# nighting0le01/On_Device_Image_Captioning

Measured on AMD Instinct MI355X. Metric: captions/sec end-to-end (Swin-L 384, beam=3) at 1/2/4/8 MI355X, higher is better.
Workload: dtype bf16; 1 GPU; End_ExpansionNet_v2 end-to-end, Swin-L/384 backbone, batch 16 per GPU, beam 3, beam_max_seq_len 20 (BASELINE.json configs[2]); workload_key=e2e16, batch_per_gpu=16, beam=3, beam_max_seq_len=20, decoder_steps=19, weights=synthetic xavier (Philox, seed 0), backbone_precision=bf16, encoder_precision=bf16, decoder_precision=fp32, hip_graphs=True, parallelism=image-shard x1, caption_len_check=20, encode_lanes=1, decode_lanes=2, decode_cus=0, decode_group_batches=1

## Files before the change

include/odic_hip.h:

```cpp
#ifndef ODIC_HIP_H
#define ODIC_HIP_H

#include <stddef.h>
#include <stdint.h>

#ifdef __cplusplus
extern "C" {
#endif

#define ODIC_F32 0
#define ODIC_BF16 1
#define ODIC_FP8 2
#define ODIC_F16 3
#define ODIC_H2 4

#define ODIC_ACT_NONE 0
#define ODIC_ACT_GELU 1
#define ODIC_ACT_RELU 2
#define ODIC_ACT_SIGMOID 3

#define ODIC_EINVAL (-1)
#define ODIC_ENULL (-2)
#define ODIC_EUNSUPPORTED (-3)

#define ODIC_ABI_VERSION 22
int odic_abi_version(void);

const char* odic_build_info(void);

typedef struct odic_gemm_args {
  const void* A; const void* W; const float* bias; const float* residual; void* out;
  int32_t M, N, K;
  int64_t lda, ldw, ldr, ldc;
  int32_t batch;
  int64_t strideA, strideW, strideBias, strideR, strideC;
  float alpha;
  int32_t act;
  int32_t bias_axis;
  int32_t in_dtype;
  int32_t out_dtype;
  int32_t tile_cfg;
  const float* ln_colsum; float ln_eps;
  int32_t* workspace;
  const float* col_scale; float out_scale;
  void* out16; int64_t ld16; float* stats_out;
  const float* ln_stats;
  const float* a_ln; int64_t ld_aln;
} odic_gemm_args;
int odic_gemm(const odic_gemm_args* args, void* stream);

int odic_layernorm(const float* x, int64_t ldx, const float* gamma, const float* beta, void* out,
                   int32_t M, int32_t C, float eps, int32_t out_dtype, void* stream);

int odic_copy(const void* src, void* dst, int64_t nbytes, void* stream);

int odic_cast_f32_to_bf16(const float* x, int64_t ldx, void* out, int64_t ldo, int32_t M, int32_t C,
                          void* stream);
int odic_cast_f32_to_h2(const float* x, int64_t ldx, void* out, int64_t ldo, int32_t M, int32_t C, void* stream);

int odic_patch_merge_layernorm(const float* x, const float* gamma, const float* beta, void* out,
                               int32_t B, int32_t res, int32_t C, float eps, int32_t out_dtype,
                               void* stream);

int odic_patch_embed(const float* img, const float* w, const float* b, const float* gamma,
                     const float* beta, float* out, int32_t B, int32_t in_chans, int32_t H,
                     int32_t W, int32_t patch, int32_t C, float eps, void* stream);

int odic_resize_bilinear_normalize(const uint8_t* src_rgb, int32_t H, int32_t W, int64_t src_stride_bytes,
                                   const int32_t* bounds_x, const int32_t* coef_x, int32_t ksize_x,
                                   const int32_t* bounds_y, const int32_t* coef_y, int32_t ksize_y,
                                   uint8_t* tmp, float* dst, int32_t out_size, const float* mean3,
                                   const float* std3, void* stream);

typedef struct odic_resize_job {
  int64_t src_off, src_pitch, tmp_off;
  int32_t H, W, row_first, n_rows;
  int32_t bounds_x, coef_x, bounds_y, coef_y;
  int32_t ksize_x, ksize_y;
// ... 36 lines not shown
#define ODIC_JPEG_MAX_SCANS 64

typedef struct odic_jpeg_table {
  uint16_t lut[512];
  int32_t maxcode[18];
  int32_t valoff[18];
  uint8_t huffval[256];
} odic_jpeg_table;

typedef struct odic_jpeg_prog_header {
  int64_t out_off, coef_off, plane_off;
  int32_t width, height, sampling, mcus_x, mcus_y, n_intervals;
  uint16_t qt[3][64];
} odic_jpeg_prog_header;

typedef struct odic_jpeg_scan {
  int64_t data_off, data_end, scan_off;
  int32_t image, int_off, n_intervals, restart, n_units, blocks_w, comp_mask, ss, se, ah, al, level;
  int32_t table[3];
  int32_t pad;
} odic_jpeg_scan;

typedef struct odic_jpeg_prog_batch {
  const void* headers;
  const void* scans;
  const void* tables;
  const uint8_t* data;
  uint8_t* out;
  int32_t* status;
  int32_t n_images, n_scans, n_tables, n_levels, max_width, max_height, pad0, pad1;
  int64_t max_blocks, total_scan_bytes, total_intervals, total_blocks, total_plane_bytes;
  int32_t level_first[ODIC_JPEG_MAX_SCANS + 1];
  int32_t level_intervals[ODIC_JPEG_MAX_SCANS];
  int32_t pad2;
} odic_jpeg_prog_batch;

size_t odic_jpeg_progressive_workspace_bytes(const odic_jpeg_prog_batch* batch);

size_t odic_jpeg_progressive_coef_offset(const odic_jpeg_prog_batch* batch);

int odic_jpeg_decode_progressive(const odic_jpeg_prog_batch* batch, void* workspace, size_t ws_bytes, void* stream);

int odic_jpeg_decode_progressive_scaled(const odic_jpeg_prog_batch* batch, const int32_t* scale_log2, void* workspace,
                                        size_t ws_bytes, void* stream);

int odic_window_attention(const void* qkv, const float* bias_table, const float* bias_shifted_prescaled,
                          void* out, int32_t B, int32_t res, int32_t C, int32_t heads, int32_t ws,
                          int32_t shift, float scale, int32_t dtype, void* stream);

int odic_swin_qkv_attention(const float* x, int64_t ldx, const void* w_qkv_folded, const float* b_qkv_folded,
                            const float* bias_shifted_prescaled, void* out, int32_t B, int32_t res, int32_t C,
                            int32_t heads, int32_t ws, int32_t shift, float scale, float ln_eps, void* stream);

int odic_stcexp_normalize(const float* z, const int32_t* enc_len, const int32_t* group_meta,
                          int32_t ngroups, void* pos_fw, void* neg_fw, int64_t ld_fw, void* pos_bw,
                          void* neg_bw, int64_t ld_bw, float* colsum_ws, int32_t B, int32_t nq,
                          int32_t S, float eps, float scale_fw, float scale_bw, int32_t out_dtype, void* stream);

int odic_selector_mix(const float* x, int64_t ldx, const float* sel_pre, int64_t lds,
                      const float* a, int64_t lda, const float* b, int64_t ldb, float* out,
                      int64_t ldo, int32_t M, int32_t d, void* stream);


int odic_dec_embed(const int64_t* tokens, const float* embed, const float* pos_table,
                   const int32_t* pos, float* y, int64_t ldy, int32_t N, int32_t d, int32_t pos_rows,
                   float scale, void* stream);

int odic_dynexp_step(const float* lin, int64_t ldlin, const float* qexp, const float* bexp,
                     float* cond_c, float* key_c, float* va_c, float* vb_c, float* wfa_c,
                     float* wfb_c, float* qk_c, const int32_t* anc, const int32_t* row_valid,
                     const int32_t* pos, const float* y_in, int64_t ldy_in, float* y, int64_t ldy,
                     int32_t N, int32_t T, int32_t d, int32_t E, float eps, void* stream);


int odic_dec_embed_seq(const int64_t* tokens, const float* embed, const float* pos_table, const int32_t* dec_len,
                       int32_t* row_valid, float* y, int64_t ldy, int32_t N, int32_t T, int32_t d, int32_t vocab,
                       int32_t pos_rows, float scale, void* stream);

int odic_dynexp_seq(const float* lin, int64_t ldlin, const float* qexp, const float* bexp, const int32_t* dec_len,
                    const float* y_in, int64_t ldy_in, float* y, int64_t ldy, int32_t N, int32_t T, int32_t d,
                    int32_t E, float eps, void* stream);

int odic_token_stats(const float* logits, int64_t ldl, const int64_t* target, float* logp_target, float* sum_logp,
                     int32_t* argmax, float* max_logp, int32_t* status, int32_t R, int32_t V, void* stream);

int odic_cross_attn_step(const float* q, int64_t ldq, const float* kv, int64_t ldkv, int32_t koff,
                         int32_t voff, const int32_t* enc_len, const int32_t* row_valid, float* out,
                         int64_t ldo, int32_t N, int32_t n_img, int32_t S, int32_t d, int32_t heads,
                         void* stream);

int odic_cross_attn_probs(const float* q, int64_t ldq, const float* kv, int64_t ldkv, int32_t koff,
                          const int32_t* enc_len, const int32_t* row_valid, float* out, int64_t ldo,
                          int32_t N, int32_t n_img, int32_t S, int32_t d, int32_t heads,
                          int32_t per_head, int32_t accumulate, float scale, void* stream);

int odic_logsoftmax_topk(const float* logits, int64_t ldl, float* logp_out, int64_t ldp,
                         float* top_val, int32_t* top_idx, int32_t N, int32_t V, int32_t k,
                         void* stream);

int odic_logsoftmax_sample(const float* logits, int64_t ldl, float* logp_out, int64_t ldp, float* top_val,
                           int32_t* top_idx, int32_t N, int32_t V, int32_t k, uint64_t seed,
                           const int32_t* pos, void* stream);

int odic_ensemble_logprobs(const float* const* logits, int32_t M, int64_t ldl, float* out, int64_t ldo,
                           int32_t N, int32_t V, void* stream);
int odic_topk_rows(const float* logp, int64_t ldl, float* top_val, int32_t* top_idx, int32_t N, int32_t V,
// ... 30 lines not shown
```

on_device_image_captioning_amd/_hip.py:

```python
from __future__ import annotations

import ctypes as C
import os

_HERE = os.path.dirname(os.path.abspath(__file__))
LIB_PATH = os.path.join(_HERE, "libodic_hip.so")

F32, BF16, FP8, F16, H2 = 0, 1, 2, 3, 4
ACT_NONE, ACT_GELU, ACT_RELU, ACT_SIGMOID = 0, 1, 2, 3
ABI_VERSION = 22

_ERR = {-1: "ODIC_EINVAL (bad shape / alignment / enum)", -2: "ODIC_ENULL (required pointer is NULL)",
        -3: "ODIC_EUNSUPPORTED"}


class GemmArgs(C.Structure):
    _fields_ = [("A", C.c_void_p), ("W", C.c_void_p), ("bias", C.c_void_p), ("residual", C.c_void_p),
                ("out", C.c_void_p),
                ("M", C.c_int32), ("N", C.c_int32), ("K", C.c_int32),
                ("lda", C.c_int64), ("ldw", C.c_int64), ("ldr", C.c_int64), ("ldc", C.c_int64),
                ("batch", C.c_int32),
                ("strideA", C.c_int64), ("strideW", C.c_int64), ("strideBias", C.c_int64),
                ("strideR", C.c_int64), ("strideC", C.c_int64),
                ("alpha", C.c_float), ("act", C.c_int32), ("bias_axis", C.c_int32),
                ("in_dtype", C.c_int32), ("out_dtype", C.c_int32), ("tile_cfg", C.c_int32),
                ("ln_colsum", C.c_void_p), ("ln_eps", C.c_float), ("workspace", C.c_void_p),
                ("col_scale", C.c_void_p), ("out_scale", C.c_float),
                ("out16", C.c_void_p), ("ld16", C.c_int64), ("stats_out", C.c_void_p), ("ln_stats", C.c_void_p),
                ("a_ln", C.c_void_p), ("ld_aln", C.c_int64)]


class BeamState(C.Structure):
    _fields_ = [(n, C.c_void_p) for n in
                ("tokens", "logprobs", "anc", "cumul", "n_elem", "has_eos", "row_valid", "next_tok",
                 "pos", "done", "ctr")]


class EmbedArgs(C.Structure):
    _fields_ = [("embed", C.c_void_p), ("pos_table", C.c_void_p), ("y", C.c_void_p), ("ldy", C.c_int64),
                ("d", C.c_int32), ("scale", C.c_float), ("pos_rows", C.c_int32)]


class JpegBatch(C.Structure):
    _fields_ = [("headers", C.c_void_p), ("data", C.c_void_p), ("out", C.c_void_p), ("status", C.c_void_p),
                ("n_images", C.c_int32), ("subseq_bits", C.c_int32), ("max_sync_passes", C.c_int32),
                ("max_units", C.c_int32), ("max_intervals", C.c_int32), ("max_width", C.c_int32),
                ("max_height", C.c_int32), ("pad", C.c_int32),
                ("max_blocks", C.c_int64), ("max_scan_bytes", C.c_int64), ("total_scan_bytes", C.c_int64),
                ("total_intervals", C.c_int64), ("total_units", C.c_int64), ("total_blocks", C.c_int64),
                ("total_plane_bytes", C.c_int64)]


JPEG_MAX_SCANS = 64


class JpegProgBatch(C.Structure):
    _fields_ = [("headers", C.c_void_p), ("scans", C.c_void_p), ("tables", C.c_void_p), ("data", C.c_void_p),
                ("out", C.c_void_p), ("status", C.c_void_p),
                ("n_images", C.c_int32), ("n_scans", C.c_int32), ("n_tables", C.c_int32), ("n_levels", C.c_int32),
                ("max_width", C.c_int32), ("max_height", C.c_int32), ("pad0", C.c_int32), ("pad1", C.c_int32),
                ("max_blocks", C.c_int64), ("total_scan_bytes", C.c_int64), ("total_intervals", C.c_int64),
                ("total_blocks", C.c_int64), ("total_plane_bytes", C.c_int64),
                ("level_first", C.c_int32 * (JPEG_MAX_SCANS + 1)), ("level_intervals", C.c_int32 * JPEG_MAX_SCANS),
                ("pad2", C.c_int32)]


_P, _I32, _I64, _F = C.c_void_p, C.c_int32, C.c_int64, C.c_float

_SIGNATURES = {
    "odic_abi_version": (C.c_int, []),
    "odic_build_info": (C.c_char_p, []),
    "odic_gemm": (C.c_int, [C.POINTER(GemmArgs), _P]),
    "odic_layernorm": (C.c_int, [_P, _I64, _P, _P, _P, _I32, _I32, _F, _I32, _P]),
    "odic_cast_f32_to_bf16": (C.c_int, [_P, _I64, _P, _I64, _I32, _I32, _P]),
    "odic_cast_f32_to_h2": (C.c_int, [_P, _I64, _P, _I64, _I32, _I32, _P]),
    "odic_patch_merge_layernorm": (C.c_int, [_P, _P, _P, _P, _I32, _I32, _I32, _F, _I32, _P]),
    "odic_patch_embed": (C.c_int, [_P] * 6 + [_I32] * 6 + [_F, _P]),
    "odic_resize_bilinear_normalize": (C.c_int, [_P, _I32, _I32, _I64, _P, _P, _I32, _P, _P, _I32, _P, _P, _I32,
                                                 C.POINTER(C.c_float), C.POINTER(C.c_float), _P]),
    "odic_resize_boxes_normalize": (C.c_int, [_P, _I32, _P, _P, _P, _P, C.c_size_t, _P, _I32, _I32,
                                              C.POINTER(C.c_float), C.POINTER(C.c_float), _P]),
    "odic_window_attention": (C.c_int, [_P, _P, _P, _P] + [_I32] * 6 + [_F, _I32, _P]),
    "odic_swin_qkv_attention": (C.c_int, [_P, _I64, _P, _P, _P, _P] + [_I32] * 6 + [_F, _F, _P]),
    "odic_stcexp_normalize": (C.c_int, [_P, _P, _P, _I32, _P, _P, _I64, _P, _P, _I64, _P, _I32, _I32, _I32, _F, _F, _F, _I32,
                                        _P]),
    "odic_selector_mix": (C.c_int, [_P, _I64, _P, _I64, _P, _I64, _P, _I64, _P, _I64, _I32, _I32, _P]),
    "odic_copy": (C.c_int, [_P, _P, _I64, _P]),
    "odic_dec_embed": (C.c_int, [_P, _P, _P, _P, _P, _I64, _I32, _I32, _I32, _F, _P]),
    "odic_dec_embed_seq": (C.c_int, [_P, _P, _P, _P, _P, _P, _I64] + [_I32] * 5 + [_F, _P]),
    "odic_dynexp_seq": (C.c_int, [_P, _I64, _P, _P, _P, _P, _I64, _P, _I64] + [_I32] * 4 + [_F, _P]),
    "odic_token_stats": (C.c_int, [_P, _I64, _P, _P, _P, _P, _P, _P, _I32, _I32, _P]),
    "odic_dynexp_step": (C.c_int, [_P, _I64, _P, _P] + [_P] * 7 + [_P, _P, _P, _P, _I64, _P, _I64] + [_I32] * 4 + [_F, _P]),
    "odic_cross_attn_step": (C.c_int, [_P, _I64, _P, _I64, _I32, _I32, _P, _P, _P, _I64] + [_I32] * 5 + [_P]),
    "odic_cross_attn_probs": (C.c_int, [_P, _I64, _P, _I64, _I32, _P, _P, _P, _I64] + [_I32] * 7 + [_F, _P]),
    "odic_logsoftmax_topk": (C.c_int, [_P, _I64, _P, _I64, _P, _P, _I32, _I32, _I32, _P]),
    "odic_logsoftmax_sample": (C.c_int, [_P, _I64, _P, _I64, _P, _P, _I32, _I32, _I32, C.c_uint64, _P, _P]),
    "odic_ensemble_logprobs": (C.c_int, [C.POINTER(C.c_void_p), _I32, _I64, _P, _I64, _I32, _I32, _P]),
    "odic_topk_rows": (C.c_int, [_P, _I64, _P, _P, _I32, _I32, _I32, _P]),
    "odic_beam_step": (C.c_int, [_P, _P, C.POINTER(BeamState), C.POINTER(EmbedArgs), _I32, _I32, _I32, _I64, _P]),
    "odic_beam_finalize": (C.c_int, [C.POINTER(BeamState), _P, _P, _I32, _I32, _P]),
    "odic_beam_finalize_best": (C.c_int, [C.POINTER(BeamState), _P, _P, _P, _P, _I32, _I32, _I32, _I32, _P]),
    "odic_beam_reset": (C.c_int, [C.POINTER(BeamState), C.POINTER(EmbedArgs), _I32, _I32, _I32, _I64, _P]),
    "odic_jpeg_workspace_bytes": (C.c_size_t, [C.POINTER(JpegBatch)]),
    "odic_jpeg_decode": (C.c_int, [C.POINTER(JpegBatch), _P, C.c_size_t, _P]),
    "odic_jpeg_progressive_workspace_bytes": (C.c_size_t, [C.POINTER(JpegProgBatch)]),
    "odic_jpeg_progressive_coef_offset": (C.c_size_t, [C.POINTER(JpegProgBatch)]),
    "odic_jpeg_decode_progressive": (C.c_int, [C.POINTER(JpegProgBatch), _P, C.c_size_t, _P]),
    "odic_jpeg_decode_scaled": (C.c_int, [C.POINTER(JpegBatch), _P, _P, C.c_size_t, _P]),
    "odic_jpeg_decode_progressive_scaled": (C.c_int, [C.POINTER(JpegProgBatch), _P, _P, C.c_size_t, _P]),
}

EXPORTED_SYMBOLS = tuple(_SIGNATURES)

_lib = None


def load() -> C.CDLL:
    global _lib
    if _lib is not None:
        return _lib
    if not os.path.exists(LIB_PATH):
        raise RuntimeError(
            f"{LIB_PATH} is missing: the HIP extension is not built and there is no CPU fallback. "
            "Run `python -c 'import __graft_entry__ as g; g.build()'` from the repository root.")
    lib = C.CDLL(LIB_PATH)
    for name, (res, args) in _SIGNATURES.items():
        fn = getattr(lib, name)
        fn.restype = res
        fn.argtypes = args
    got = lib.odic_abi_version()
    if got != ABI_VERSION:
        raise RuntimeError(f"libodic_hip.so ABI {got} != binding ABI {ABI_VERSION}; rebuild")
    _lib = lib
    return lib


# ... 7 lines not shown
```

on_device_image_captioning_amd/csrc/gemm_bf16.hip:

```cpp
#include "gemm_tile.h"
#include <stdio.h>
#include <stdlib.h>
#include <type_traits>

namespace {

struct Params {
  const bf16_raw* A; const bf16_raw* W; const float* bias; const float* residual; void* out;
  int M, N, K;
  long lda, ldw, ldr, ldc;
  long strideA, strideW, strideBias, strideR, strideC;
  float alpha; int act; int bias_axis;
  TileGrid grid;
  const float* a_ln; long ld_aln; float ln_eps;
};

template <int NWM, int NWN, int MI, int NI, int NSTAGE, int BK, typename OutT, int KS = 1>
__global__ __launch_bounds__(64 * NWM * NWN * KS, (NWM * NWN * KS == 4 && MI * NI == 32) ? 2 : 1) void gemm_bf16_nt_kernel(Params p) {
  static_assert(KS == 1 || (KS == 2 && BK == 64), "the K-split form is two groups on 64-deep K-tiles");
  constexpr int NW = NWM * NWN;
  constexpr int ROWB = BK * 2;
  constexpr int RPI = 1024 / ROWB;
  constexpr int CPR = ROWB / 16;
  constexpr int BM = NWM * MI * 16, BN = NWN * NI * 16;
// ... 514 lines not shown
    } else {
#pragma unroll
      for (int nq = 0; nq < NI / 2; ++nq) {
#pragma unroll
        for (int mi = 0; mi < MI; ++mi) {
          f32x4_t v[2];
          finish(mi, nq, v);
          OutT* dst = out + (long)(m0 + (wave * MI + mi) * 16 + frow) * p.ldc + c * BNC + nq * 32 + fq * 8;
          if constexpr (sizeof(OutT) == 4) {
            ((f32x4_t*)dst)[0] = v[0]; ((f32x4_t*)dst)[1] = v[1];
          } else {
            bf16x8_t pk;
#pragma unroll
            for (int e = 0; e < 4; ++e) { pk[e] = (short)f32_to_bf16(v[0][e]); pk[4 + e] = (short)f32_to_bf16(v[1][e]); }
            *(bf16x8_t*)dst = pk;
          }
        }
      }
    }
  }
}

template <int MI, int NI, int KT, int KH = 1>
int launch_apanel(Params& p, int out_dtype, int batch, hipStream_t stream) {
  constexpr int BM = 4 * MI * 16, BNC = NI * 16;
  if (batch != 1 || p.K != KT * 64 || p.M % BM != 0 || p.N % BNC != 0 || p.bias_axis != 0)
    return ODIC_EUNSUPPORTED;
  if ((long)BNC * p.ldw >= (1L << 30) || (p.residual && MI > 2))
    return ODIC_EUNSUPPORTED;
  if ((p.ldc & 7) || ((uintptr_t)p.out & 15) || (p.residual && ((p.ldr & 3) || ((uintptr_t)p.residual & 15))))
    return ODIC_EUNSUPPORTED;
  const int panels = p.M / BM, nchunks = p.N / BNC;
  static const int want = getenv("ODIC_APANEL_BLOCKS") ? atoi(getenv("ODIC_APANEL_BLOCKS")) : 1536;
  const int nsplit = panel_split(panels, nchunks, want);
  dim3 grid(8 * ((panels + 7) / 8) * nsplit), block(256);
  const int SHMEM = 2 * (KT / KH) * BNC * 128 + (nchunks + nsplit - 1) / nsplit * BNC * 4;
  if (SHMEM > 64 * 1024) return ODIC_EUNSUPPORTED;
  if (p.a_ln) {
    if (p.residual || (p.ld_aln & 3) || ((uintptr_t)p.a_ln & 15)) return ODIC_EUNSUPPORTED;
    if (out_dtype == ODIC_BF16) hipLaunchKernelGGL((gemm_bf16_apanel_kernel<MI, NI, KT, KH, bf16_raw, false, true>), grid, block, SHMEM, stream, p, nsplit);
    else hipLaunchKernelGGL((gemm_bf16_apanel_kernel<MI, NI, KT, KH, float, false, true>), grid, block, SHMEM, stream, p, nsplit);
    return odic_launch_status();
  }
  if constexpr (MI <= 2) {
    if (p.residual) {
      if (out_dtype == ODIC_BF16) hipLaunchKernelGGL((gemm_bf16_apanel_kernel<MI, NI, KT, KH, bf16_raw, true>), grid, block, SHMEM, stream, p, nsplit);
      else hipLaunchKernelGGL((gemm_bf16_apanel_kernel<MI, NI, KT, KH, float, true>), grid, block, SHMEM, stream, p, nsplit);
      return odic_launch_status();
    }
  }
  if (out_dtype == ODIC_BF16) hipLaunchKernelGGL((gemm_bf16_apanel_kernel<MI, NI, KT, KH, bf16_raw, false>), grid, block, SHMEM, stream, p, nsplit);
  else hipLaunchKernelGGL((gemm_bf16_apanel_kernel<MI, NI, KT, KH, float, false>), grid, block, SHMEM, stream, p, nsplit);
  return odic_launch_status();
}

template <int NWM, int NWN, int MI, int NI, int NSTAGE, int BK = 64, int KS = 1>
int launch_cfg(Params& p, int out_dtype, int batch, hipStream_t stream) {
  constexpr int BM = NWM * MI * 16, BN = NWN * NI * 16;
  constexpr int SH_STAGES = NSTAGE * (BM + BN) * BK * 2 + BM * 8;
  constexpr int SH_RED = KS == 2 ? NWM * NWN * MI * NI * 1024 : 0;
  constexpr int SHMEM = SH_STAGES > SH_RED ? SH_STAGES : SH_RED;
  if (p.K % BK != 0) return ODIC_EINVAL;
  const int max_rect = tile_grid(p.grid, p.M, p.N, BM, BN, (double)p.M * p.K * 2.0, (double)p.N * p.K * 2.0,
                                 32 * (NWM * NWN * KS <= 4 ? 2 : 1));
  dim3 grid(8 * max_rect, 1, batch), block(64 * NWM * NWN * KS);
  constexpr auto kb = gemm_bf16_nt_kernel<NWM, NWN, MI, NI, NSTAGE, BK, bf16_raw, KS>;
  constexpr auto kf = gemm_bf16_nt_kernel<NWM, NWN, MI, NI, NSTAGE, BK, float, KS>;
  tile_allow_lds<SHMEM, kb, kf>();
  if (out_dtype == ODIC_BF16) hipLaunchKernelGGL(kb, grid, block, SHMEM, stream, p);
  else hipLaunchKernelGGL(kf, grid, block, SHMEM, stream, p);
  return odic_launch_status();
}


}

int odic_gemm_bf16_launch(const odic_gemm_args* a, hipStream_t stream) {
  if (a->ln_colsum) return ODIC_EUNSUPPORTED;
  if (a->K % 64 != 0 || (a->A && a->lda % 8 != 0) || a->ldw % 8 != 0) return ODIC_EINVAL;
  if (((uintptr_t)a->A & 15) || ((uintptr_t)a->W & 15)) return ODIC_EINVAL;
  if (a->a_ln && (a->tile_cfg < 50 || a->tile_cfg > 53)) return ODIC_EUNSUPPORTED;
  if (!a->a_ln && !a->A) return ODIC_EINVAL;
  if ((a->strideA % 8) || (a->strideW % 8)) return ODIC_EINVAL;
  Params p;
  p.A = (const bf16_raw*)a->A; p.W = (const bf16_raw*)a->W; p.bias = a->bias; p.residual = a->residual;
  p.out = a->out; p.M = a->M; p.N = a->N; p.K = a->K;
  p.lda = a->lda; p.ldw = a->ldw; p.ldr = a->ldr; p.ldc = a->ldc;
  p.strideA = a->strideA; p.strideW = a->strideW; p.strideBias = a->strideBias;
  p.strideR = a->strideR; p.strideC = a->strideC;
  p.alpha = a->alpha; p.act = a->act; p.bias_axis = a->bias_axis;
  p.a_ln = a->a_ln; p.ld_aln = a->ld_aln; p.ln_eps = a->ln_eps;
  int cfg = a->tile_cfg;
  if (cfg < 0) {
    const double c0 = tile_rounds(a->M, a->N, a->batch, 128, 64, 768) * 1.0;
    const double c1 = tile_rounds(a->M, a->N, a->batch, 128, 128, 512) * 1.38;
    const double c2 = a->N % 256 == 0 ? tile_rounds(a->M, a->N, a->batch, 256, 256, 256) * 2.6 : 1e30;
    cfg = (c0 <= c1 && c0 <= c2) ? 0 : (c1 <= c2 ? 1 : 2);
  }
  switch (cfg) {
    case 0: return launch_cfg<2, 2, 4, 2, 2>(p, a->out_dtype, a->batch, stream);
    case 1: return launch_cfg<2, 2, 4, 4, 2>(p, a->out_dtype, a->batch, stream);
    case 2: return launch_cfg<2, 4, 8, 4, 2>(p, a->out_dtype, a->batch, stream);
    case 7: return launch_cfg<4, 2, 4, 4, 2, 32>(p, a->out_dtype, a->batch, stream);
    case 10: return launch_cfg<4, 2, 4, 4, 3, 32>(p, a->out_dtype, a->batch, stream);
    case 40: return launch_cfg<6, 2, 3, 6, 2, 64>(p, a->out_dtype, a->batch, stream);
    case 41: return launch_cfg<3, 3, 3, 6, 2, 64>(p, a->out_dtype, a->batch, stream);
    case 42: return launch_cfg<3, 2, 3, 6, 2, 64>(p, a->out_dtype, a->batch, stream);
    case 43: return launch_cfg<3, 2, 3, 6, 3, 64>(p, a->out_dtype, a->batch, stream);
    case 44: return launch_cfg<3, 1, 3, 6, 2, 64>(p, a->out_dtype, a->batch, stream);
    case 45: return launch_cfg<3, 3, 3, 6, 3, 32>(p, a->out_dtype, a->batch, stream);
    case 46: return launch_cfg<3, 1, 3, 6, 3, 64>(p, a->out_dtype, a->batch, stream);
    case 47: return launch_cfg<3, 2, 3, 6, 2, 64, 2>(p, a->out_dtype, a->batch, stream);
    case 48: return launch_cfg<2, 2, 2, 2, 3, 64>(p, a->out_dtype, a->batch, stream);
    case 49: return launch_cfg<2, 2, 2, 2, 2, 64>(p, a->out_dtype, a->batch, stream);
    case 50: return launch_apanel<4, 4, 3>(p, a->out_dtype, a->batch, stream);
    case 51: return launch_apanel<2, 2, 6>(p, a->out_dtype, a->batch, stream);
    case 52: return launch_apanel<2, 4, 3>(p, a->out_dtype, a->batch, stream);
    case 53: return launch_apanel<2, 4, 6, 2>(p, a->out_dtype, a->batch, stream);
    default: return ODIC_EINVAL;
  }
}
```

on_device_image_captioning_amd/engine.py:

```python
from __future__ import annotations

import ctypes as C
import math
import os
from typing import Dict, List, Optional, Sequence, Tuple

import torch

from . import _hip, ops
from .weights import Geometry

SD = Dict[str, torch.Tensor]
_CDT = {"fp32": torch.float32, "bf16": torch.bfloat16, "fp8": torch.bfloat16, "x3": ops.H2_DTYPE}


def pack_operand(t: torch.Tensor, cdt) -> Tuple[torch.Tensor, float]:
    if cdt == ops.H2_DTYPE:
        sc = ops.pow2_scale_for_h2(t)
        return ops.h2_from_f32(t * sc), 1.0 / sc
    return t.to(cdt).contiguous(), 1.0


def _dev(t: torch.Tensor, device, dtype=None) -> torch.Tensor:
    t = t.detach()
    if dtype is not None and t.dtype != dtype:
        t = t.to(dtype)
    return t.to(device).contiguous()


class SwinEngine:
    def __init__(self, sd: SD, g: Geometry, device, precision: str = "fp32", calibration_images=None):
        if precision not in _CDT:
            raise ValueError(f"precision must be one of {list(_CDT)}")
        self.g, self.device, self.precision = g, device, precision
        self.cdt = _CDT[precision]
        fp8 = precision == "fp8"
        fast_attn = precision in ("bf16", "fp8", "x3")
        P = "swin_transf"
        f32 = lambda k: _dev(sd[k], device, torch.float32)
        cw = lambda k: pack_operand(_dev(sd[k], device, torch.float32), self.cdt)
        self.pe_w = _dev(sd[f"{P}.patch_embed.proj.weight"].reshape(g.swin_embed_dim, -1), device, torch.float32)
        self.pe_b = f32(f"{P}.patch_embed.proj.bias")
        self.pe_g, self.pe_beta = f32(f"{P}.patch_embed.norm.weight"), f32(f"{P}.patch_embed.norm.bias")
        self.stages = []
        for s, depth in enumerate(g.swin_depths):
            blocks = []
            for b in range(depth):
                p = f"{P}.layers.{s}.blocks.{b}"
                (qkv_w, qkv_a), (proj_w, proj_a) = cw(p + ".attn.qkv.weight"), cw(p + ".attn.proj.weight")
                (fc1_w, fc1_a), (fc2_w, fc2_a) = cw(p + ".mlp.fc1.weight"), cw(p + ".mlp.fc2.weight")
                blocks.append(dict(
                    n1w=f32(p + ".norm1.weight"), n1b=f32(p + ".norm1.bias"),
                    qkv_w=qkv_w, qkv_a=qkv_a, qkv_b=f32(p + ".attn.qkv.bias"),
                    table=f32(p + ".attn.relative_position_bias_table"),
                    dense=(ops.shifted_bias_prescaled(f32(p + ".attn.relative_position_bias_table"), g.stage_window(s),
                                                      (g.stage_dim(s) // g.swin_num_heads[s]) ** -0.5)
                           if fast_attn and g.stage_window(s) == 12 else None),
                    proj_w=proj_w, proj_a=proj_a, proj_b=f32(p + ".attn.proj.bias"),
                    n2w=f32(p + ".norm2.weight"), n2b=f32(p + ".norm2.bias"),
                    fc1_w=fc1_w, fc1_a=fc1_a, fc1_b=f32(p + ".mlp.fc1.bias"),
                    fc2_w=fc2_w, fc2_a=fc2_a, fc2_b=f32(p + ".mlp.fc2.bias"),
                    shift=g.stage_shift(s, b)))
            down = None
            if s < len(g.swin_depths) - 1:
                p = f"{P}.layers.{s}.downsample"
                red_w, red_a = cw(p + ".reduction.weight")
                down = dict(nw=f32(p + ".norm.weight"), nb=f32(p + ".norm.bias"), red_w=red_w, red_a=red_a)
            self.stages.append((blocks, down))
        self.fn_w, self.fn_b = f32(f"{P}.norm.weight"), f32(f"{P}.norm.bias")
        self.stage_chunks = [int(v) for v in os.environ.get("ODIC_SWIN_CHUNKS", "1").split(",")]
        lr = os.environ.get("ODIC_FUSE_BACKBONE_LN_READ", "1")
        self.ln_read = (precision == "bf16" and lr != "0") or (precision == "x3" and lr == "x3")
        self.fuse_qkv_attn = precision == "bf16" and os.environ.get("ODIC_FUSE_QKV_ATTENTION", "1") == "1"
        if self.ln_read:
            for s, (blocks, _) in enumerate(self.stages):
                if g.stage_dim(s) != 192:
                    continue
                for b, w in enumerate(blocks):
                    p = f"{P}.layers.{s}.blocks.{b}"
                    if precision == "bf16":
                        w["qkv_lnr"] = ops.fold_layernorm_bf16(f32(p + ".attn.qkv.weight"), w["qkv_b"], w["n1w"], w["n1b"])[:2] + (1.0,)
                        w["fc1_lnr"] = ops.fold_layernorm_bf16(f32(p + ".mlp.fc1.weight"), w["fc1_b"], w["n2w"], w["n2b"])[:2] + (1.0,)
                    else:
                        for name, wk, bk, nw, nb in (("qkv_lnr", ".attn.qkv.weight", "qkv_b", "n1w", "n1b"),
                                                     ("fc1_lnr", ".mlp.fc1.weight", "fc1_b", "n2w", "n2b")):
                            Wg, b2, _ = ops.fold_layernorm(f32(p + wk), w[bk], w[nw], w[nb])
                            op, alpha = pack_operand(Wg, self.cdt)
                            w[name] = (op, b2, alpha)
        self.fp8_ready = False
        if fp8:
            self._pack_fp8(sd, calibration_images)

    def _pack_fp8(self, sd: SD, calibration_images) -> None:
        from .weights import synth_images
        g, dv = self.g, self.device
        if any(g.stage_window(s) != 12 or g.stage_dim(s) % 64 for s in range(len(g.swin_depths))):
            raise RuntimeError("fp8 mode needs 12x12 windows and stage widths that are multiples of 64 (Swin-L: 192·2^s)")
        img = calibration_images if calibration_images is not None else synth_images(2, g, seed=7)
        amax = {}
        self.forward(img.to(dv, torch.float32), _amax=amax)
        P = "swin_transf"
        margin = 1.25
        self.fp8_range = {k: margin * v for k, v in amax.items()}
        for s, (blocks, _) in enumerate(self.stages):
            for b, w in enumerate(blocks):
                p = f"{P}.layers.{s}.blocks.{b}"
                s1 = margin * amax[(s, b, "ln1")] / ops.FP8_MAX
                s2 = margin * amax[(s, b, "ln2")] / ops.FP8_MAX
                sh = margin * amax[(s, b, "hid")] / ops.FP8_MAX
                f32 = lambda k: _dev(sd[k], dv, torch.float32)
                q_qkv, sw_qkv = ops.quantize_fp8_per_channel(f32(p + ".attn.qkv.weight"))
                q_fc1, sw_fc1 = ops.quantize_fp8_per_channel(f32(p + ".mlp.fc1.weight"))
                q_fc2, sw_fc2 = ops.quantize_fp8_per_channel(f32(p + ".mlp.fc2.weight"))
                w.update(dict(
                    n1w8=(w["n1w"] / s1).contiguous(), n1b8=(w["n1b"] / s1).contiguous(),
                    n2w8=(w["n2w"] / s2).contiguous(), n2b8=(w["n2b"] / s2).contiguous(),
                    qkv_w8=q_qkv, qkv_cs=(sw_qkv * s1).contiguous(),
                    fc1_w8=q_fc1, fc1_cs=(sw_fc1 * s2).contiguous(), hid_inv=1.0 / sh,
                    fc2_w8=q_fc2, fc2_cs=(sw_fc2 * sh).contiguous(),
                    proj_w16=f32(p + ".attn.proj.weight").to(torch.float16).contiguous()))
        self.fp8_ready = True

    def fp8_saturation(self, img: torch.Tensor) -> dict:
        if not self.fp8_ready:
            raise RuntimeError("not an fp8 engine")
        seen = {}
        self.forward(img, _amax=seen)
        ratios = {k: seen[k] / self.fp8_range[k] for k in seen}
        over = {f"s{k[0]}b{k[1]}.{k[2]}": round(v, 3) for k, v in ratios.items() if v > 1.0}
        return {"tensors": len(ratios), "clipping_tensors": len(over), "worst_ratio": round(max(ratios.values()), 3),
                "median_ratio": round(sorted(ratios.values())[len(ratios) // 2], 3), "clipping": over}

    def forward(self, img: torch.Tensor, taps: Optional[dict] = None, out_dtype=torch.float32,
                _amax: Optional[dict] = None) -> torch.Tensor:
        g, cdt = self.g, self.cdt
        if img.dtype != torch.float32 or not img.is_cuda:
            raise RuntimeError("SwinEngine.forward wants an fp32 CUDA image batch")
        img = img.contiguous()
        B = img.shape[0]
        fp8 = self.fp8_ready and _amax is None
        x = ops.patch_embed(img, self.pe_w, self.pe_b, self.pe_g, self.pe_beta, g.swin_patch_size)
        if taps is not None:
            taps["patch_embed"] = x.clone()
        for s, (blocks, down) in enumerate(self.stages):
            res, C_, heads, ws = g.stage_res(s), g.stage_dim(s), g.swin_num_heads[s], g.stage_window(s)
            x = x.view(B * res * res, C_)
            n_ch = self.stage_chunks[s] if s < len(self.stage_chunks) else 1
            if taps is not None or _amax is not None or n_ch < 1 or B % n_ch:
                n_ch = 1
            x_all, B_all = x, B
            B = B_all // n_ch
            for ci, bi, w in ((ci, bi, w) for ci in range(n_ch) for bi, w in enumerate(blocks)):
                x = x_all[ci * B * res * res:(ci + 1) * B * res * res]
                if fp8:
                    xn = ops.layernorm(x, w["n1w8"], w["n1b8"], out_dtype=ops.FP8_DTYPE)
                    qkv = ops.gemm(xn, w["qkv_w8"], w["qkv_b"], col_scale=w["qkv_cs"], out_dtype=torch.float16)
                    att = ops.window_attention(qkv, w["table"], B, res, C_, heads, ws, w["shift"],
                                               bias_shifted_prescaled=w["dense"])
                    ops.gemm(att, w["proj_w16"], w["proj_b"], residual=x, out=x)
                    xn = ops.layernorm(x, w["n2w8"], w["n2b8"], out_dtype=ops.FP8_DTYPE)
                    h = ops.gemm(xn, w["fc1_w8"], w["fc1_b"], act=ops.ACT_GELU, col_scale=w["fc1_cs"],
                                 out_scale=w["hid_inv"], out_dtype=ops.FP8_DTYPE)
                    ops.gemm(h, w["fc2_w8"], w["fc2_b"], residual=x, out=x, col_scale=w["fc2_cs"])
                elif "qkv_lnr" in w and _amax is None and ops.a_ln_supported(x.shape[0], 3 * C_, C_, cdt):
                    if self.fuse_qkv_attn and ws == 12 and w["dense"] is not None:
                        att = ops.swin_qkv_attention(x, w["qkv_lnr"][0], w["qkv_lnr"][1], w["dense"], B, res, C_, heads,
                                                     ws, w["shift"])
                    else:
                        qkv = ops.gemm(None, w["qkv_lnr"][0], w["qkv_lnr"][1], a_ln=x, out_dtype=cdt, alpha=w["qkv_lnr"][2])
                        att = ops.window_attention(qkv, w["table"], B, res, C_, heads, ws, w["shift"],
                                                   bias_shifted_prescaled=w["dense"])
                    ops.gemm(att, w["proj_w"], w["proj_b"], residual=x, out=x, alpha=w["proj_a"])
                    h = ops.gemm(None, w["fc1_lnr"][0], w["fc1_lnr"][1], a_ln=x, act=ops.ACT_GELU, out_dtype=cdt,
                                 alpha=w["fc1_lnr"][2])
                    ops.gemm(h, w["fc2_w"], w["fc2_b"], residual=x, out=x, alpha=w["fc2_a"])
                else:
                    xn = ops.layernorm(x, w["n1w"], w["n1b"], out_dtype=cdt)
                    if _amax is not None:
                        _amax[(s, bi, "ln1")] = float(xn.float().abs().max())
                    qkv = ops.gemm(xn, w["qkv_w"], w["qkv_b"], alpha=w["qkv_a"])
                    att = ops.window_attention(qkv, w["table"], B, res, C_, heads, ws, w["shift"],
                                               bias_shifted_prescaled=w["dense"])
                    ops.gemm(att, w["proj_w"], w["proj_b"], residual=x, out=x, alpha=w["proj_a"])
                    xn = ops.layernorm(x, w["n2w"], w["n2b"], out_dtype=cdt)
                    h = ops.gemm(xn, w["fc1_w"], w["fc1_b"], act=ops.ACT_GELU, alpha=w["fc1_a"])
                    if _amax is not None:
                        _amax[(s, bi, "ln2")] = float(xn.float().abs().max())
                        _amax[(s, bi, "hid")] = float(h.float().abs().max())
                    ops.gemm(h, w["fc2_w"], w["fc2_b"], residual=x, out=x, alpha=w["fc2_a"])
                if taps is not None:
                    taps[f"s{s}b{bi}"] = x.view(B, res * res, C_).clone()
            x, B = x_all, B_all
            if down is not None:
                xm = ops.patch_merge_layernorm(x, down["nw"], down["nb"], B, res, C_, out_dtype=cdt)
                x = ops.gemm(xm.view(-1, 4 * C_), down["red_w"], out_dtype=torch.float32, alpha=down["red_a"])
                if taps is not None:
                    taps[f"merge{s}"] = x.view(B, (res // 2) ** 2, 2 * C_).clone()
        res = g.stage_res(len(g.swin_depths) - 1)
        out = ops.layernorm(x, self.fn_w, self.fn_b, out_dtype=out_dtype)
        return out.view(B, res * res, -1)


class DecodeState:

    def __init__(self, eng: "CaptionerEngine", n_img: int, beams: int, T: int, kv: torch.Tensor,
                 enc_len: torch.Tensor, S: int):
        g, dv = eng.g, eng.device
        N = n_img * beams
        d, E, L = g.d_model, g.num_exp_dec, g.N_dec
        self.n_img, self.beams, self.N, self.T, self.S = n_img, beams, N, T, S
        self.kv, self.enc_len = kv, enc_len
        f = lambda *s: torch.zeros(*s, dtype=torch.float32, device=dv)
        i32 = lambda *s: torch.zeros(*s, dtype=torch.int32, device=dv)
        self.ycat = f(N, L * d)
        self.caches = [dict(cond=f(T, N, d), key=f(T, N, d), va=f(T, N, d), vb=f(T, N, d),
                            wfa=f(T, N, T, E), wfb=f(T, N, T, E), qk=f(T, N, E)) for _ in range(L)]
        self.anc = i32(N, T)
        self.row_valid = torch.ones(N, dtype=torch.int32, device=dv)
        self.next_tok = torch.zeros(N, dtype=torch.int64, device=dv)
        self.pos, self.done, self.ctr = i32(1), i32(1), i32(1)
        self.tokens = torch.zeros(n_img, beams, T, dtype=torch.int64, device=dv)
        self.logprobs = f(n_img, beams, T)
        self.cumul, self.n_elem, self.has_eos = f(N), i32(N), i32(N)
        self.cand_val, self.cand_idx = f(N, beams), i32(N, beams)
        self.logits = f(N, g.vocab_size)
        self.beam_state = _hip.BeamState(*(t.data_ptr() for t in (
            self.tokens, self.logprobs, self.anc, self.cumul, self.n_elem, self.has_eos, self.row_valid,
            self.next_tok, self.pos, self.done, self.ctr)))
# ... 305 lines not shown
```

on_device_image_captioning_amd/ops.py:

```python
from __future__ import annotations

import ctypes as C
import os
from typing import Optional, Sequence

import torch

from . import _hip
from ._hip import ACT_GELU, ACT_NONE, ACT_RELU, ACT_SIGMOID, BF16, F16, F32, FP8, H2

FP8_DTYPE = torch.float8_e4m3fn
FP8_MAX = 448.0
H2_DTYPE = torch.int32
_DT = {torch.float32: F32, torch.bfloat16: BF16, torch.float16: F16, FP8_DTYPE: FP8, H2_DTYPE: H2}


def _stream() -> C.c_void_p:
    return C.c_void_p(torch.cuda.current_stream().cuda_stream)


_PROFILE: Optional[list] = None


class profile:
# ... 325 lines not shown
    _need_cuda(x, gamma, beta)
    out = torch.empty((B, (res // 2) ** 2, 4 * Cin), dtype=out_dtype, device=x.device)
    with _timed("patch_merge_layernorm", 8.0 * out.numel(), out.numel() * (4 + out.element_size())):
        _hip.check(_hip.load().odic_patch_merge_layernorm(_p(x), _p(gamma), _p(beta), _p(out), B, res, Cin, eps,
                                                          dtype_code(out_dtype), _stream()),
                   "odic_patch_merge_layernorm")
    return out


def patch_embed(img: torch.Tensor, w: torch.Tensor, b: torch.Tensor, gamma: torch.Tensor, beta: torch.Tensor,
                patch: int, *, eps: float = 1e-5) -> torch.Tensor:
    _need_cuda(img, w, b, gamma, beta)
    B, Cin, H, Wd = img.shape
    Cout = w.shape[0]
    if not img.is_contiguous() or img.dtype != torch.float32:
        raise RuntimeError("patch_embed: image batch must be contiguous fp32 [B,C,H,W]")
    out = torch.empty((B, (H // patch) * (Wd // patch), Cout), dtype=torch.float32, device=img.device)
    with _timed("patch_embed", 2.0 * out.numel() * Cin * patch * patch, (img.numel() + out.numel()) * 4):
        _hip.check(_hip.load().odic_patch_embed(_p(img), _p(w), _p(b), _p(gamma), _p(beta), _p(out), B, Cin, H, Wd,
                                                patch, Cout, eps, _stream()), "odic_patch_embed")
    return out


def shifted_bias_prescaled(bias_table: torch.Tensor, ws: int, scale: float) -> torch.Tensor:
    if ws != 12:
        raise RuntimeError("the packed bias layout is specialised for 12x12 windows")
    heads = bias_table.shape[1]
    t = (bias_table.double() / scale).float().view(23, 23, heads)
    R = torch.zeros(heads, 23 * 24 + 32, dtype=torch.float32, device=bias_table.device)
    R[:, :23 * 24].view(heads, 23, 24)[:, :, :23] = t.flip(1).permute(2, 0, 1)
    out = torch.zeros(heads, 4, 576, dtype=torch.float32, device=bias_table.device)
    for s_ in range(4):
        out[:, s_, :] = R[:, s_:s_ + 576]
    return out.contiguous()


def swin_qkv_attention(x: torch.Tensor, w_folded: torch.Tensor, b_folded: torch.Tensor, bias_shifted_prescaled: torch.Tensor,
                       B: int, res: int, C_: int, heads: int, ws: int, shift: int, *, eps: float = 1e-5,
                       out: Optional[torch.Tensor] = None) -> torch.Tensor:
    _need_cuda(x, w_folded, b_folded, bias_shifted_prescaled, out)
    if x.dtype != torch.float32 or w_folded.dtype != torch.bfloat16 or not (x.is_contiguous() and w_folded.is_contiguous()):
        raise RuntimeError("swin_qkv_attention: contiguous fp32 rows and a contiguous bf16 folded weight")
    if out is None:
        out = torch.empty(B * res * res, C_, dtype=torch.bfloat16, device=x.device)
    nwh = B * (res // ws) ** 2 * heads
    with _timed("swin_qkv_attention", 2.0 * B * res * res * C_ * 3 * C_ + nwh * 2654208.0,
                B * res * res * C_ * (4 + 2) + 3 * C_ * C_ * 2, f"res{res}h{heads}"):
        _hip.check(_hip.load().odic_swin_qkv_attention(_p(x), C_, _p(w_folded), _p(b_folded), _p(bias_shifted_prescaled),
                                                      _p(out), B, res, C_, heads, ws, shift, (C_ // heads) ** -0.5, eps,
                                                      _stream()), "odic_swin_qkv_attention")
    return out


def window_attention(qkv: torch.Tensor, bias_table: torch.Tensor, B: int, res: int, C_: int, heads: int, ws: int,
                     shift: int, *, scale: Optional[float] = None, out: Optional[torch.Tensor] = None,
                     bias_shifted_prescaled: Optional[torch.Tensor] = None) -> torch.Tensor:
    _need_cuda(qkv, bias_table, out, bias_shifted_prescaled)
    if scale is None:
        scale = (C_ // heads) ** -0.5
    if out is None:
        out = torch.empty((B * res * res, C_), dtype=qkv.dtype, device=qkv.device)
    inst = B * (res // ws) ** 2 * heads
    n = ws * ws
    fam = ("window_attention_bf16" if qkv.dtype in (torch.bfloat16, torch.float16) else
           "window_attention_x3" if qkv.dtype == H2_DTYPE else "window_attention_f32")
    with _timed(fam, inst * 4.0 * n * n * 32, inst * 4.0 * n * 32 * qkv.element_size(), f"res{res}h{heads}"):
        _hip.check(_hip.load().odic_window_attention(_p(qkv), _p(bias_table), _p(bias_shifted_prescaled), _p(out), B, res, C_,
                                                     heads, ws, shift,
                                                     scale, dtype_code(qkv.dtype), _stream()),
                   "odic_window_attention")
    return out


def stcexp_group_meta(groups: Sequence[int], device) -> torch.Tensor:
    starts = [0]
    gid = []
    for g, n in enumerate(groups):
        starts.append(starts[-1] + n)
        gid += [g] * n
    return torch.tensor(starts + gid, dtype=torch.int32, device=device)


def stcexp_normalize(z: torch.Tensor, enc_len: torch.Tensor, group_meta: torch.Tensor, ngroups: int,
                     pos_fw: torch.Tensor, neg_fw: torch.Tensor, pos_bw: torch.Tensor, neg_bw: torch.Tensor,
                     colsum_ws: torch.Tensor, *, eps: float = 1e-9, scale_fw: float = 1.0, scale_bw: float = 1.0) -> None:
    _need_cuda(z, enc_len, group_meta, pos_fw, neg_fw, pos_bw, neg_bw, colsum_ws)
    B, nq, S = z.shape
    osz = pos_fw.element_size()
    with _timed("stcexp_normalize", 6.0 * B * nq * S,
                B * nq * S * 4.0 + 2.0 * B * nq * pos_fw.shape[-1] * osz + 2.0 * B * S * pos_bw.shape[-1] * osz):
        _hip.check(_hip.load().odic_stcexp_normalize(_p(z), _p(enc_len), _p(group_meta), ngroups, _p(pos_fw),
                                                     _p(neg_fw), pos_fw.shape[-1], _p(pos_bw), _p(neg_bw),
                                                     pos_bw.shape[-1], _p(colsum_ws), B, nq, S, eps, scale_fw, scale_bw,
                                                     dtype_code(pos_fw.dtype), _stream()), "odic_stcexp_normalize")


def selector_mix(x, ldx, sel_pre, lds, a, lda, b, ldb, out, ldo, M, d) -> None:
    _need_cuda(x, sel_pre, a, b, out)
    with _timed("selector_mix", 6.0 * M * d, 5.0 * M * d * 4):
        _hip.check(_hip.load().odic_selector_mix(_p(x), ldx, _p(sel_pre), lds, _p(a), lda, _p(b), ldb, _p(out), ldo,
                                                 M, d, _stream()), "odic_selector_mix")


def dec_embed(tokens, embed, pos_table, pos, y, ldy, N, d, scale) -> None:
    _need_cuda(tokens, embed, pos_table, pos, y)
    with _timed("dec_embed", 2.0 * N * d, N * (8.0 + 2 * d * 4) + d * 4):
# ... 138 lines not shown
```

Before: 1915 captions/s.

## Fuse Swin MLP (LN, fc1, GELU, fc2, residual) into one kernel

Adds a HIP kernel for the C=192 Swin stage. It applies the row layernorm in registers, runs fc1 in 64-column hidden chunks, applies GELU, and feeds each chunk straight into fc2 accumulators before adding bias and residual. The 4C-wide hidden activation is never written to global memory, and two GEMM launches become one. Weight chunks for fc1 and fc2 are streamed into LDS with double-issued direct-to-LDS loads so the copies overlap the MFMA work. In exchange, each block recomputes with only four waves and a fixed tile shape. The fc1 alpha is hardcoded to 1, which is only correct if the folded weights already include it.

```diff
diff --git a/include/odic_hip.h b/include/odic_hip.h
--- a/include/odic_hip.h
+++ b/include/odic_hip.h
@@ -23,7 +23,7 @@
 #define ODIC_ENULL (-2)
 #define ODIC_EUNSUPPORTED (-3)
 
-#define ODIC_ABI_VERSION 22
+#define ODIC_ABI_VERSION 23
 int odic_abi_version(void);
 
 const char* odic_build_info(void);
@@ -166,6 +166,10 @@
                             const float* bias_shifted_prescaled, void* out, int32_t B, int32_t res, int32_t C,
                             int32_t heads, int32_t ws, int32_t shift, float scale, float ln_eps, void* stream);
 
+int odic_swin_mlp(const float* x, int64_t ldx, const void* w1_folded, const float* b1_folded, const void* w2,
+                  const float* b2, float alpha2, float* out, int64_t ldo, int32_t M, int32_t C, float ln_eps,
+                  void* stream);
+
 int odic_stcexp_normalize(const float* z, const int32_t* enc_len, const int32_t* group_meta,
                           int32_t ngroups, void* pos_fw, void* neg_fw, int64_t ld_fw, void* pos_bw,
                           void* neg_bw, int64_t ld_bw, float* colsum_ws, int32_t B, int32_t nq,
diff --git a/on_device_image_captioning_amd/_hip.py b/on_device_image_captioning_amd/_hip.py
--- a/on_device_image_captioning_amd/_hip.py
+++ b/on_device_image_captioning_amd/_hip.py
@@ -8,7 +8,7 @@
 
 F32, BF16, FP8, F16, H2 = 0, 1, 2, 3, 4
 ACT_NONE, ACT_GELU, ACT_RELU, ACT_SIGMOID = 0, 1, 2, 3
-ABI_VERSION = 22
+ABI_VERSION = 23
 
 _ERR = {-1: "ODIC_EINVAL (bad shape / alignment / enum)", -2: "ODIC_ENULL (required pointer is NULL)",
         -3: "ODIC_EUNSUPPORTED"}
@@ -82,6 +82,7 @@
                                               C.POINTER(C.c_float), C.POINTER(C.c_float), _P]),
     "odic_window_attention": (C.c_int, [_P, _P, _P, _P] + [_I32] * 6 + [_F, _I32, _P]),
     "odic_swin_qkv_attention": (C.c_int, [_P, _I64, _P, _P, _P, _P] + [_I32] * 6 + [_F, _F, _P]),
+    "odic_swin_mlp": (C.c_int, [_P, _I64, _P, _P, _P, _P, _F, _P, _I64, _I32, _I32, _F, _P]),
     "odic_stcexp_normalize": (C.c_int, [_P, _P, _P, _I32, _P, _P, _I64, _P, _P, _I64, _P, _I32, _I32, _I32, _F, _F, _F, _I32,
                                         _P]),
     "odic_selector_mix": (C.c_int, [_P, _I64, _P, _I64, _P, _I64, _P, _I64, _P, _I64, _I32, _I32, _P]),
diff --git a/on_device_image_captioning_amd/csrc/gemm_bf16.hip b/on_device_image_captioning_amd/csrc/gemm_bf16.hip
--- a/on_device_image_captioning_amd/csrc/gemm_bf16.hip
+++ b/on_device_image_captioning_amd/csrc/gemm_bf16.hip
@@ -590,6 +590,194 @@
   if (out_dtype == ODIC_BF16) hipLaunchKernelGGL((gemm_bf16_apanel_kernel<MI, NI, KT, KH, bf16_raw, false>), grid, block, SHMEM, stream, p, nsplit);
   else hipLaunchKernelGGL((gemm_bf16_apanel_kernel<MI, NI, KT, KH, float, false>), grid, block, SHMEM, stream, p, nsplit);
   return odic_launch_status();
+}
+
+struct MlpParams {
+  const float* x; float* out; const bf16_raw* W1; const float* b1; const bf16_raw* W2; const float* b2;
+  long ldx, ldo; int M;
+  float alpha1, alpha2, ln_eps;
+};
+
+template <int MI, int KT>
+__global__ __launch_bounds__(256, 2) void swin_mlp_kernel(MlpParams p) {
+  constexpr int NW = 4;
+  constexpr int C = KT * 64, H = 4 * C, BM = NW * MI * 16;
+  constexpr int NO = C / 16;
+  constexpr int SUB = 64 * 128;
+  constexpr int W1B = KT * SUB, W2B = C * 128;
+  constexpr int I1 = W1B / 1024 / NW, I2 = W2B / 1024 / NW;
+  static_assert(W1B % (1024 * NW) == 0 && W2B % (1024 * NW) == 0, "a chunk must split into whole DMA instructions per wave");
+  extern __shared__ __attribute__((aligned(16))) char lds[];
+
+  const int tid = threadIdx.x, lane = tid & 63, wave = tid >> 6;
+  ODIC_ENCODE_PRIO();
+  const int m0 = blockIdx.x * BM;
+  float alpha1_v = p.alpha1, alpha2_v = p.alpha2;
+  asm volatile("" : "+v"(alpha1_v), "+v"(alpha2_v));
+  const int frow = lane & 15, fq = lane >> 4;
+
+  int w1_off[I1], w2_off[I2];
+  {
+    const int srow = lane >> 3, sch = swz<128>(lane & 7, srow) * 8;
+#pragma unroll
+    for (int i = 0; i < I1; ++i) {
+      const int j = i * NW + wave, kt = j / 8, rg = j - kt * 8;
+      w1_off[i] = wperm(rg * 8 + srow) * C + kt * 64 + sch;
+    }
+#pragma unroll
+    for (int i = 0; i < I2; ++i) w2_off[i] = wperm((i * NW + wave) * 8 + srow) * H + sch;
+  }
+  char* const l1 = lds;
+  char* const l2 = lds + W1B;
+  auto issue1 = [&](int c) {
+    const bf16_raw* wb = p.W1 + (long)c * 64 * C;
+#pragma unroll
+    for (int i = 0; i < I1; ++i)
+      __builtin_amdgcn_global_load_lds((gptr_t)(wb + w1_off[i]), (lptr_t)(l1 + (i * NW + wave) * 1024), 16, 0, 0);
+  };
+  auto issue2 = [&](int c) {
+    const bf16_raw* wb = p.W2 + c * 64;
+#pragma unroll
+    for (int i = 0; i < I2; ++i)
+      __builtin_amdgcn_global_load_lds((gptr_t)(wb + w2_off[i]), (lptr_t)(l2 + (i * NW + wave) * 1024), 16, 0, 0);
+  };
+  issue1(0);
+  float* sb1 = (float*)(lds + W1B + W2B);
+  float* sb2 = sb1 + H;
+  for (int t = tid; t < H; t += 256) sb1[t] = p.b1[t];
+  for (int t = tid; t < C; t += 256) sb2[t] = p.b2[t];
+
+  bf16x8_t af[2 * KT][MI];
+#pragma unroll
+  for (int mi = 0; mi < MI; ++mi) {
+    const float* xr = p.x + (long)(m0 + (wave * MI + mi) * 16 + frow) * p.ldx + fq * 8;
+    f32x4_t xv[2 * KT][2];
+#pragma unroll
+    for (int k = 0; k < 2 * KT; ++k) { xv[k][0] = *(const f32x4_t*)(xr + k * 32); xv[k][1] = *(const f32x4_t*)(xr + k * 32 + 4); }
+    f32x4_t s4 = {0.f, 0.f, 0.f, 0.f};
+#pragma unroll
+    for (int k = 0; k < 2 * KT; ++k) s4 += xv[k][0] + xv[k][1];
+    float sum = (s4[0] + s4[1]) + (s4[2] + s4[3]);
+    sum += __shfl_xor(sum, 16, 64);
+    sum += __shfl_xor(sum, 32, 64);
+    const float mean = sum / (float)(64 * KT);
+    f32x4_t q4 = {0.f, 0.f, 0.f, 0.f};
+#pragma unroll
+    for (int k = 0; k < 2 * KT; ++k) {
+      xv[k][0] -= mean; xv[k][1] -= mean;
+      q4 += xv[k][0] * xv[k][0] + xv[k][1] * xv[k][1];
+    }
+    float ssq = (q4[0] + q4[1]) + (q4[2] + q4[3]);
+    ssq += __shfl_xor(ssq, 16, 64);
+    ssq += __shfl_xor(ssq, 32, 64);
+    const float rstd = rsqrtf(ssq / (float)(64 * KT) + p.ln_eps);
+#pragma unroll
+    for (int k = 0; k < 2 * KT; ++k) {
+      bf16x8_t f;
+#pragma unroll
+      for (int e = 0; e < 4; ++e) {
+        f[e] = (short)f32_to_bf16(xv[k][0][e] * rstd);
+        f[4 + e] = (short)f32_to_bf16(xv[k][1][e] * rstd);
+      }
+      af[k][mi] = f;
+    }
+  }
+
+  f32x4_t acc2[MI][NO];
+#pragma unroll
+  for (int i = 0; i < MI; ++i)
+#pragma unroll
+    for (int j = 0; j < NO; ++j) acc2[i][j] = f32x4_t{0.f, 0.f, 0.f, 0.f};
+
+  __builtin_amdgcn_s_waitcnt(0x0070);
+  const char* lw1 = l1 + frow * 128;
+  const char* lw2 = l2 + frow * 128;
+  for (int c = 0; c < H / 64; ++c) {
+    __builtin_amdgcn_s_waitcnt(0x0F70);
+    __builtin_amdgcn_s_barrier();
+    issue2(c);
+    f32x4_t acc1[MI][4];
+#pragma unroll
+    for (int i = 0; i < MI; ++i)
+#pragma unroll
+      for (int j = 0; j < 4; ++j) acc1[i][j] = f32x4_t{0.f, 0.f, 0.f, 0.f};
+#pragma unroll
+    for (int kt = 0; kt < KT; ++kt) {
+#pragma unroll
+      for (int kk = 0; kk < 2; ++kk) {
+        bf16x8_t wf[4];
+        const int chunk = swz<128>(kk * 4 + fq, frow) << 4;
+#pragma unroll
+        for (int ni = 0; ni < 4; ++ni) wf[ni] = *(const bf16x8_t*)(lw1 + kt * SUB + ni * 16 * 128 + chunk);
+#pragma unroll
+        for (int mi = 0; mi < MI; ++mi)
+#pragma unroll
+          for (int ni = 0; ni < 4; ++ni)
+            acc1[mi][ni] = __builtin_amdgcn_mfma_f32_16x16x32_bf16(wf[ni], af[2 * kt + kk][mi], acc1[mi][ni], 0, 0, 0);
+      }
+    }
+    bf16x8_t hf[2][MI];
+#pragma unroll
+    for (int mi = 0; mi < MI; ++mi) {
+#pragma unroll
+      for (int q = 0; q < 2; ++q) {
+        const f32x4_t* sb = (const f32x4_t*)(sb1 + c * 64 + q * 32 + fq * 8);
+        bf16x8_t f;
+#pragma unroll
+        for (int h = 0; h < 2; ++h) {
+          f32x4_t pre = acc1[mi][2 * q + h] * alpha1_v + sb[h];
+          pre = gelu_poly4(pre);
+#pragma unroll
+          for (int e = 0; e < 4; ++e) f[4 * h + e] = (short)f32_to_bf16(pre[e]);
+        }
+        hf[q][mi] = f;
+      }
+    }
+    __builtin_amdgcn_s_waitcnt(0x0F70);
+    __builtin_amdgcn_s_barrier();
+    if (c + 1 < H / 64) issue1(c + 1);
+#pragma unroll
+    for (int kk = 0; kk < 2; ++kk) {
+      const int chunk = swz<128>(kk * 4 + fq, frow) << 4;
+#pragma unroll
+      for (int n4 = 0; n4 < NO / 4; ++n4) {
+        bf16x8_t wf[4];
+#pragma unroll
+        for (int ni = 0; ni < 4; ++ni) wf[ni] = *(const bf16x8_t*)(lw2 + (n4 * 4 + ni) * 16 * 128 + chunk);
+#pragma unroll
+        for (int mi = 0; mi < MI; ++mi)
+#pragma unroll
+          for (int ni = 0; ni < 4; ++ni)
+            acc2[mi][n4 * 4 + ni] = __builtin_amdgcn_mfma_f32_16x16x32_bf16(wf[ni], hf[kk][mi], acc2[mi][n4 * 4 + ni], 0, 0, 0);
+      }
+    }
+  }
+
+  constexpr int NG = NO / 2;
+  const float brow = 0.f;
+  f32x4_t rv[2][MI][2];
+  auto loadg = [&](int q, int slot) {
+#pragma unroll
+    for (int mi = 0; mi < MI; ++mi) {
+      const f32x4_t* rp = (const f32x4_t*)(p.x + (long)(m0 + (wave * MI + mi) * 16 + frow) * p.ldx + q * 32 + fq * 8);
+      rv[slot][mi][0] = rp[0]; rv[slot][mi][1] = rp[1];
+    }
+  };
+  loadg(0, 0);
+#pragma unroll
+  for (int q = 0; q < NG; ++q) {
+    if (q + 1 < NG) loadg(q + 1, (q + 1) & 1);
+    const f32x4_t* sb = (const f32x4_t*)(sb2 + q * 32 + fq * 8);
+#pragma unroll
+    for (int mi = 0; mi < MI; ++mi) {
+      f32x4_t v[2];
+#pragma unroll
+      for (int h = 0; h < 2; ++h) v[h] = acc2[mi][2 * q + h] * alpha2_v + sb[h] + brow;
+      v[0] += rv[q & 1][mi][0]; v[1] += rv[q & 1][mi][1];
+      float* dst = p.out + (long)(m0 + (wave * MI + mi) * 16 + frow) * p.ldo + q * 32 + fq * 8;
+      ((f32x4_t*)dst)[0] = v[0]; ((f32x4_t*)dst)[1] = v[1];
+    }
+  }
 }
 
 template <int NWM, int NWN, int MI, int NI, int NSTAGE, int BK = 64, int KS = 1>
@@ -658,3 +846,20 @@
     default: return ODIC_EINVAL;
   }
 }
+
+extern "C" int odic_swin_mlp(const float* x, int64_t ldx, const void* w1_folded, const float* b1_folded, const void* w2,
+                             const float* b2, float alpha2, float* out, int64_t ldo, int32_t M, int32_t C, float ln_eps,
+                             void* stream) {
+  if (!x || !w1_folded || !b1_folded || !w2 || !b2 || !out) return ODIC_ENULL;
+  constexpr int MI = 2, BM = 4 * MI * 16;
+  if (C != 192 || M <= 0 || M % BM != 0) return ODIC_EINVAL;
+  if (ldx < C || ldo < C || (ldx & 3) || (ldo & 3)) return ODIC_EINVAL;
+  if (((uintptr_t)x & 15) || ((uintptr_t)out & 15) || ((uintptr_t)w1_folded & 15) || ((uintptr_t)w2 & 15)) return ODIC_EINVAL;
+  MlpParams p;
+  p.x = x; p.out = out; p.W1 = (const bf16_raw*)w1_folded; p.b1 = b1_folded; p.W2 = (const bf16_raw*)w2; p.b2 = b2;
+  p.ldx = ldx; p.ldo = ldo; p.M = M;
+  p.alpha1 = 1.0f; p.alpha2 = alpha2; p.ln_eps = ln_eps;
+  const int SHMEM = 2 * 64 * C * 2 + 5 * C * 4;
+  hipLaunchKernelGGL((swin_mlp_kernel<MI, 3>), dim3(M / BM), dim3(256), SHMEM, (hipStream_t)stream, p);
+  return odic_launch_status();
+}
diff --git a/on_device_image_captioning_amd/engine.py b/on_device_image_captioning_amd/engine.py
--- a/on_device_image_captioning_amd/engine.py
+++ b/on_device_image_captioning_amd/engine.py
@@ -72,6 +72,7 @@
         lr = os.environ.get("ODIC_FUSE_BACKBONE_LN_READ", "1")
         self.ln_read = (precision == "bf16" and lr != "0") or (precision == "x3" and lr == "x3")
         self.fuse_qkv_attn = precision == "bf16" and os.environ.get("ODIC_FUSE_QKV_ATTENTION", "1") == "1"
+        self.fuse_mlp = precision == "bf16" and os.environ.get("ODIC_FUSE_MLP", "1") == "1"
         if self.ln_read:
             for s, (blocks, _) in enumerate(self.stages):
                 if g.stage_dim(s) != 192:
@@ -171,9 +172,12 @@
                         att = ops.window_attention(qkv, w["table"], B, res, C_, heads, ws, w["shift"],
                                                    bias_shifted_prescaled=w["dense"])
                     ops.gemm(att, w["proj_w"], w["proj_b"], residual=x, out=x, alpha=w["proj_a"])
-                    h = ops.gemm(None, w["fc1_lnr"][0], w["fc1_lnr"][1], a_ln=x, act=ops.ACT_GELU, out_dtype=cdt,
-                                 alpha=w["fc1_lnr"][2])
-                    ops.gemm(h, w["fc2_w"], w["fc2_b"], residual=x, out=x, alpha=w["fc2_a"])
+                    if self.fuse_mlp and ops.swin_mlp_supported(x.shape[0], C_, cdt):
+                        ops.swin_mlp(x, w["fc1_lnr"][0], w["fc1_lnr"][1], w["fc2_w"], w["fc2_b"], w["fc2_a"], out=x)
+                    else:
+                        h = ops.gemm(None, w["fc1_lnr"][0], w["fc1_lnr"][1], a_ln=x, act=ops.ACT_GELU, out_dtype=cdt,
+                                     alpha=w["fc1_lnr"][2])
+                        ops.gemm(h, w["fc2_w"], w["fc2_b"], residual=x, out=x, alpha=w["fc2_a"])
                 else:
                     xn = ops.layernorm(x, w["n1w"], w["n1b"], out_dtype=cdt)
                     if _amax is not None:
diff --git a/on_device_image_captioning_amd/ops.py b/on_device_image_captioning_amd/ops.py
--- a/on_device_image_captioning_amd/ops.py
+++ b/on_device_image_captioning_amd/ops.py
@@ -401,6 +401,31 @@
     return out
 
 
+def swin_mlp_supported(M: int, C_: int, dtype=torch.bfloat16) -> bool:
+    return dtype == torch.bfloat16 and C_ == 192 and M > 0 and M % 128 == 0
+
+
+def swin_mlp(x: torch.Tensor, w1_folded: torch.Tensor, b1_folded: torch.Tensor, w2: torch.Tensor, b2: torch.Tensor,
+             alpha2: float = 1.0, out: Optional[torch.Tensor] = None, ln_eps: float = 1e-5) -> torch.Tensor:
+    _need_cuda(x, w1_folded, b1_folded, w2, b2, out)
+    if x.dtype != torch.float32 or w1_folded.dtype != torch.bfloat16 or w2.dtype != torch.bfloat16 or \
+            not (x.is_contiguous() and w1_folded.is_contiguous() and w2.is_contiguous()):
+        raise RuntimeError("swin_mlp: contiguous fp32 rows and contiguous bf16 weights")
+    C_ = x.shape[-1]
+    M = x.numel() // C_
+    if tuple(w1_folded.shape) != (4 * C_, C_) or tuple(w2.shape) != (C_, 4 * C_) or b1_folded.numel() != 4 * C_ or \
+            b2.numel() != C_ or b1_folded.dtype != torch.float32 or b2.dtype != torch.float32:
+        raise RuntimeError("swin_mlp: fc1 is [4C, C] with an fp32 bias [4C], fc2 [C, 4C] with an fp32 bias [C]")
+    if out is None:
+        out = torch.empty_like(x)
+    elif out.dtype != torch.float32 or out.shape != x.shape or not out.is_contiguous():
+        raise RuntimeError("swin_mlp: out is a contiguous fp32 tensor of x's shape")
+    with _timed("swin_mlp", 2.0 * M * C_ * 4 * C_ * 2, 2.0 * M * C_ * 4 + 2 * 4 * C_ * C_ * 2, f"{M}x{C_}"):
+        _hip.check(_hip.load().odic_swin_mlp(_p(x), C_, _p(w1_folded), _p(b1_folded), _p(w2), _p(b2), float(alpha2), _p(out),
+                                             C_, M, C_, float(ln_eps), _stream()), "odic_swin_mlp")
+    return out
+
+
 def window_attention(qkv: torch.Tensor, bias_table: torch.Tensor, B: int, res: int, C_: int, heads: int, ws: int,
                      shift: int, *, scale: Optional[float] = None, out: Optional[torch.Tensor] = None,
                      bias_shifted_prescaled: Optional[torch.Tensor] = None) -> torch.Tensor:
```

Result: faster. 1953 captions/s (median of 6 runs) (+2.0%).
